# TencentARC/Mix-of-Show

Measured on AMD Instinct MI355X. Metric: edlora_train_images_per_sec_512_sd15, higher is better.
Workload: dtype fp16; 1 GPU; BASELINE.json configs[1]: single-concept ED-LoRA tune, SD-1.5 UNet/CLIP/VAE (random init, calibrated), 512x512, LoRA rank 4 on Attention+CLIPAttention, attn_reg on, batch 4/GPU; global_batch=4, per_gpu_batch=4, image_size=512, parallelism=dp1, grad_bucket_bytes=4466688, preset=sd15, hipgraph=True, channels_last=True

## Files before the change

### include/mos_hip.h

```cpp
#ifndef MOS_HIP_H
#define MOS_HIP_H

#include <stdint.h>

#ifdef __cplusplus
extern "C" {
#endif

typedef enum { MOS_F16 = 0, MOS_BF16 = 1 } mos_dtype;

typedef enum {
    MOS_OK = 0,
    MOS_ERR_BAD_ARG = -1,
    MOS_ERR_UNSUPPORTED = -2,
    MOS_ERR_LAUNCH = -3
} mos_status;

#define MOS_LORA_PAD 16
#define MOS_MAX_PCOLS 4
#define MOS_MAX_SOURCES 9

int mos_version(void);
const char* mos_last_error_string(void);

// ... 66 lines not shown
                              const void* A16T, const void* BpT,
                              void* dt, void* dx, int64_t lddx,
                              const mos_lora_grad_out* grads_host, void* ws,
                              int M, int N, int K, int lora_cols, int dtype, void* stream);

typedef struct {
    const float* partial[2];
    int C[2], cb[2];
    int nchunk, nj, block_begin, n_blocks;
    mos_lora_grad_out out;
} mos_lora_final_rec;
int mos_lora_linear_fused_bwd_deferred(const void* dy, int64_t lddy, const void* x, int64_t ldx,
                                       const void* Wt, int64_t ldwt, const void* t,
                                       const void* A16T, const void* BpT,
                                       void* dt, void* dx, int64_t lddx,
                                       const mos_lora_grad_out* grads_host, void* ws,
                                       int M, int N, int K, int lora_cols, int dtype, void* stream,
                                       mos_lora_final_rec* rec_host);
int mos_lora_grad_final_all(const mos_lora_final_rec* recs_dev, int n_recs, int total_blocks, void* stream);

typedef struct {
    const void* P[2];
    const void* Z[2];
    int64_t ldz[2];
    int C[2], cb[2];
    float* partial[2];
    int M, rpc, nchunk, nj;
    int block_begin, n_blocks;
    double flops, bytes;
} mos_lora_grad_job;
int mos_lora_linear_fused_bwd_deferred_all(const void* dy, int64_t lddy, const void* x, int64_t ldx,
                                           const void* Wt, int64_t ldwt, const void* t,
                                           const void* A16T, const void* BpT,
                                           void* dt, void* dx, int64_t lddx,
                                           const mos_lora_grad_out* grads_host, void* ws,
                                           int M, int N, int K, int lora_cols, int dtype, void* stream,
                                           mos_lora_final_rec* rec_host, mos_lora_grad_job* job_host);
int mos_lora_grad_all(const mos_lora_grad_job* jobs_dev, int n_jobs, int total_blocks, int nj, int dtype, double flops, double bytes,
                      void* stream);

typedef struct {
    int B, H, Nq, Nkv, d;
    int64_t q_bs, q_rs;
    int64_t k_bs, k_rs;
    int64_t v_bs, v_rs;
    int64_t o_bs, o_rs;
    float scale;
    int causal;
} mos_attn_shape;

int mos_attn_fwd(const void* q, const void* k, const void* v, void* o, float* lse,
                 const int32_t* tok_idx, int n_pcols, float* pcols,
                 const mos_attn_shape* shape_host, int dtype, void* stream);

typedef struct {
    int64_t do_bs, do_rs;
    int64_t dq_bs, dq_rs;
    int64_t dk_bs, dk_rs;
    int64_t dv_bs, dv_rs;
} mos_attn_grad_strides;

int64_t mos_attn_bwd_workspace_bytes(const mos_attn_shape* shape_host);
int mos_attn_bwd(const void* q, const void* k, const void* v, const void* o, const float* lse,
                 const void* dO, const int32_t* tok_idx, int n_pcols, const float* pcols,
                 const float* dpcols, void* dq, void* dk, void* dv, void* ws,
                 const mos_attn_shape* shape_host, const mos_attn_grad_strides* gs_host,
                 int dtype, void* stream);

int mos_self_attn_fwd(const void* q, const void* k, const void* v, void* o, float* lse,
                      const mos_attn_shape* shape_host, int dtype, void* stream);
int mos_cross_attn_fwd(const void* q, const void* k, const void* v, void* o, float* lse,
                       const int32_t* tok_idx, int n_pcols, float* pcols,
                       const mos_attn_shape* shape_host, int dtype, void* stream);
int mos_self_attn_bwd(const void* q, const void* k, const void* v, const void* o, const float* lse, const void* dO,
                      void* dq, void* dk, void* dv, void* ws, const mos_attn_shape* shape_host,
                      const mos_attn_grad_strides* gs_host, int dtype, void* stream);
int mos_cross_attn_bwd(const void* q, const void* k, const void* v, const void* o, const float* lse, const void* dO,
                       const int32_t* tok_idx, int n_pcols, const float* pcols, const float* dpcols,
                       void* dq, void* dk, void* dv, void* ws, const mos_attn_shape* shape_host,
                       const mos_attn_grad_strides* gs_host, int dtype, void* stream);

typedef struct {
    int n_regions;
    int feat_h, feat_w;
    int box[MOS_MAX_SOURCES - 1][4];
    int64_t src_stride;
} mos_region_desc;

int mos_region_cross_attn_fwd(const void* q, const void* k_src, const void* v_src, void* o,
                              const mos_attn_shape* shape_host, const mos_region_desc* reg_host,
                              int dtype, void* stream);
int mos_region_cross_attn_fwd_chunk(const void* q, const void* k_src, const void* v_src, void* o,
                                    const mos_attn_shape* shape_host, const mos_region_desc* reg_host,
                                    const void* total_count, int accumulate, int dtype, void* stream);

int mos_attn_probs(const void* q, const void* k, void* probs, const mos_attn_shape* shape_host, int dtype, void* stream);
int mos_attn_pv(const void* probs, const void* v, void* o, const mos_attn_shape* shape_host, int dtype, void* stream);
int64_t mos_attn_probs_bwd_workspace_bytes(const mos_attn_shape* shape_host);
int mos_attn_pv_bwd(const void* probs, const void* v, const void* dO, void* dprobs, void* dv, void* ws,
                    const mos_attn_shape* shape_host, const mos_attn_grad_strides* gs_host, int dtype, void* stream);
int mos_attn_probs_bwd(const void* q, const void* k, const void* probs, const void* dprobs, void* dq, void* dk, void* ws,
                       const mos_attn_shape* shape_host, const mos_attn_grad_strides* gs_host, int dtype, void* stream);

int64_t mos_gram_workspace_bytes(int64_t n, int Cin, int Cout);
int mos_gram_accumulate(const void* X, int64_t ldx, const void* Y, int64_t ldy, int64_t n,
                        int Cin, int Cout, int dtype, double* G, double* P, double* c,
// ... 68 lines not shown
```

### mix-of-show_amd/csrc/mos_attn.hip

```cpp
#include <cstdio>
#include <cstdlib>
#include <type_traits>
#include "mos_common.h"

#ifndef MOS_DQ_OCC
#define MOS_DQ_OCC 2
#endif
#ifndef MOS_ATTN_PV16
#define MOS_ATTN_PV16 1
#endif

namespace {

constexpr float LOG2E = 1.4426950408889634f;
constexpr float NEG_BIG = -1.0e30f;
constexpr int KV_TILE = 64;
constexpr int TS = KV_TILE + 8;
__device__ __forceinline__ constexpr int tr_col(int c) { return (c & ~12) | ((c & 4) << 1) | ((c & 8) >> 1); }

__device__ __forceinline__ constexpr int tr_col16(int c) {
    return (c & 32) | ((((c >> 2) & 1) * 2 + ((c >> 4) & 1)) << 3) | (((c >> 3) & 1) << 2) | (c & 3);
}

template <int D>
// ... 1391 lines not shown

template <int D> constexpr size_t fwd_lds(size_t es) { return 2 * (HD<D>::ROW_TILE_ELEMS + HD<D>::TR_TILE_ELEMS) * es; }
template <int D> constexpr size_t dq_lds(size_t es) { return 2 * (2 * HD<D>::ROW_TILE_ELEMS + HD<D>::TR_TILE_ELEMS) * es; }
template <int D> constexpr size_t dkdv_lds(size_t es) {
    return DKDV_NBUF<D>::value * ((2 * HD<D>::ROW_TILE_ELEMS + 2 * HD<D>::TR_TILE_ELEMS) * es +
                                  KV_TILE * (2 + MOS_MAX_PCOLS) * sizeof(float));
}

template <typename K>
void set_lds(K kernel, size_t bytes) {
    if (bytes > 48 * 1024)
        (void)hipFuncSetAttribute(reinterpret_cast<const void*>(kernel), hipFuncAttributeMaxDynamicSharedMemorySize, (int)bytes);
}

int check_shape(const mos_attn_shape* s, const char* who) {
    if (!s) return mos_set_error(MOS_ERR_BAD_ARG, "%s: NULL shape", who);
    if (s->B <= 0 || s->H <= 0 || s->Nq <= 0 || s->Nkv <= 0)
        return mos_set_error(MOS_ERR_BAD_ARG, "%s: B=%d H=%d Nq=%d Nkv=%d", who, s->B, s->H, s->Nq, s->Nkv);
    if (s->d != 40 && s->d != 64 && s->d != 80 && s->d != 160)
        return mos_set_error(MOS_ERR_UNSUPPORTED, "%s: head dim %d not in {40, 64, 80, 160}", who, s->d);
    if (s->causal && s->Nq != s->Nkv)
        return mos_set_error(MOS_ERR_BAD_ARG, "%s: causal masking needs Nq == Nkv (got %d, %d)", who, s->Nq, s->Nkv);
    if (s->q_rs % 8 || s->k_rs % 8 || s->v_rs % 8 || s->o_rs % 4 || s->q_bs % 8 || s->k_bs % 8 || s->v_bs % 8 || s->o_bs % 4)
        return mos_set_error(MOS_ERR_BAD_ARG, "%s: strides must be multiples of 8 elements", who);
    return MOS_OK;
}

AttnArgs make_args(const void* q, const void* k, const void* v, void* o, float* lse, const int32_t* tok, int np,
                   float* pcols, const mos_attn_shape* s, int q_tile) {
    AttnArgs a;
    a.q = q; a.k = k; a.v = v; a.o = o; a.lse = lse; a.tok_idx = tok; a.pcols = pcols; a.n_pcols = np;
    a.B = s->B; a.H = s->H; a.Nq = s->Nq; a.Nkv = s->Nkv; a.nqb = (s->Nq + q_tile - 1) / q_tile;
    a.q_bs = s->q_bs; a.q_rs = s->q_rs; a.k_bs = s->k_bs; a.k_rs = s->k_rs;
    a.v_bs = s->v_bs; a.v_rs = s->v_rs; a.o_bs = s->o_bs; a.o_rs = s->o_rs; a.scale = s->scale;
    a.causal = s->causal;
    return a;
}

template <typename T>
const char* tname() { return sizeof(T) == 2 && std::is_same<T, f16_t>::value ? "f16" : "bf16"; }

struct AttnKey {
    char s[96];
    double flops, bytes;
    AttnKey(const char* dt, const mos_attn_shape* sh, double gemms) {
        snprintf(s, sizeof(s), "%s d%d B%d H%d Nq%d Nkv%d", dt, sh->d, sh->B, sh->H, sh->Nq, sh->Nkv);
        flops = gemms * 2.0 * sh->B * sh->H * (double)sh->Nq * sh->Nkv * sh->d;
        bytes = 2.0 * sh->B * sh->H * sh->d * (2.0 * sh->Nq + 2.0 * sh->Nkv);
    }
};

template <int D> constexpr bool has_causal() { return true; }

template <typename T, int D, int QW, bool PCOLS, bool CAUSAL>
void launch_fwd_one(const AttnArgs& a, size_t lds, hipStream_t st) {
    const dim3 grid((unsigned)(a.H * a.nqb * a.B));
    set_lds(&attn_fwd_kernel<T, D, QW, PCOLS, CAUSAL>, lds);
    hipLaunchKernelGGL((attn_fwd_kernel<T, D, QW, PCOLS, CAUSAL>), grid, dim3(256), lds, st, a);
}
template <typename T, int D, int QW>
void launch_fwd_qw(const AttnArgs& a, int np, size_t lds, hipStream_t st) {
    if constexpr (has_causal<D>()) {
        if (a.causal) {
            if (np > 0) launch_fwd_one<T, D, QW, true, true>(a, lds, st);
            else launch_fwd_one<T, D, QW, false, true>(a, lds, st);
            return;
        }
    }
    if (np > 0) launch_fwd_one<T, D, QW, true, false>(a, lds, st);
    else launch_fwd_one<T, D, QW, false, false>(a, lds, st);
}

template <typename T, int D>
int launch_fwd(const void* q, const void* k, const void* v, void* o, float* lse, const int32_t* tok, int np,
               float* pcols, const mos_attn_shape* s, hipStream_t st) {
    constexpr int QW = fwd_qw<D>();
    const size_t lds = fwd_lds<D>(sizeof(T));
    AttnKey key(tname<T>(), s, 2.0);
    MosProfScope prof(st, np > 0 ? "attn_fwd_pcols" : "attn_fwd", key.s, key.flops, key.bytes);
    const int64_t wg_big = (int64_t)s->H * s->B * ((s->Nq + 4 * QW - 1) / (4 * QW));
    if (QW == 64 && wg_big < 512) {
        launch_fwd_qw<T, D, 32>(make_args(q, k, v, o, lse, tok, np, pcols, s, 128), np, lds, st);
    } else {
        launch_fwd_qw<T, D, QW>(make_args(q, k, v, o, lse, tok, np, pcols, s, 4 * QW), np, lds, st);
    }
    return mos_check_launch("attn_fwd");
}

template <typename T, int D>
int launch_region(const void* q, const void* k, const void* v, void* o, const mos_attn_shape* s,
                  const mos_region_desc* reg, const unsigned char* total_count, int accumulate, hipStream_t st) {
    AttnArgs a = make_args(q, k, v, o, nullptr, nullptr, 0, nullptr, s, 128);
    a.nqb = ((reg->feat_w + 15) / 16) * ((reg->feat_h + 7) / 8);
    const dim3 grid((unsigned)(a.H * a.nqb * a.B));
    const size_t lds = RG<D>::lds_bytes(sizeof(T));
    set_lds(&region_attn_kernel<T, D>, lds);
    double cover = 0.0, area = 0.0;
    for (int r = 0; r < reg->n_regions; ++r) {
        const double bh = reg->box[r][2] - reg->box[r][0], bw = reg->box[r][3] - reg->box[r][1];
        if (bh > 0 && bw > 0) area += bh * bw;
    }
    cover = area + (double)s->Nq;
    AttnKey key(tname<T>(), s, 2.0);
    char rk[128];
    snprintf(rk, sizeof(rk), "%s R%d", key.s, reg->n_regions);
    MosProfScope prof(st, "region_attn", rk, key.flops * cover / (double)s->Nq, key.bytes);
    hipLaunchKernelGGL((region_attn_kernel<T, D>), grid, dim3(256), lds, st, a, *reg, total_count, accumulate);
    return mos_check_launch("region_attn");
}

struct BwdPlan { int nw_q, nw_k, nqb, nkb, nsplit, q_per_split; };
BwdPlan plan_bwd(const mos_attn_shape* s) {
    BwdPlan p;
    p.nw_q = 4;
    p.nw_k = 4;
    p.nqb = (s->Nq + 32 * p.nw_q - 1) / (32 * p.nw_q);
    p.nkb = (s->Nkv + 32 * p.nw_k - 1) / (32 * p.nw_k);
    const int64_t base = (int64_t)p.nkb * s->B * s->H;
    const int qtiles = (s->Nq + KV_TILE - 1) / KV_TILE;
    int ns = (int)((512 + base - 1) / base);
    if (ns > qtiles) ns = qtiles;
    if (ns < 1) ns = 1;
    int tps = (qtiles + ns - 1) / ns;
    ns = (qtiles + tps - 1) / tps;
    p.nsplit = ns;
    p.q_per_split = tps * KV_TILE;
    return p;
}

template <typename T, int D>
int launch_bwd(const void* q, const void* k, const void* v, const void* o, const float* lse, const void* dO,
               const int32_t* tok, int np, const float* pcols, const float* dpcols, void* dq, void* dk, void* dv,
               void* ws, const mos_attn_shape* s, const mos_attn_grad_strides* g, hipStream_t st) {
    const BwdPlan p = plan_bwd(s);
    float* Dvec = (float*)ws;
    const int64_t nrows = (int64_t)s->B * s->H * s->Nq;
    float* part = Dvec + ((nrows + 3) / 4) * 4;
    AttnBwdArgs a;
    a.q = q; a.k = k; a.v = v; a.dO = dO; a.lse = lse; a.Dvec = Dvec; a.tok_idx = tok; a.dpcols = dpcols;
    a.o = o; a.o_bs = s->o_bs; a.o_rs = s->o_rs; a.pcols = pcols;
    a.n_pcols = (dpcols != nullptr && pcols != nullptr) ? np : 0;
    a.dq = dq; a.dk = dk; a.dv = dv; a.part = part;
    a.B = s->B; a.H = s->H; a.Nq = s->Nq; a.Nkv = s->Nkv; a.nqb = p.nqb; a.nkb = p.nkb;
    a.nsplit = p.nsplit; a.q_per_split = p.q_per_split;
    a.q_bs = s->q_bs; a.q_rs = s->q_rs; a.k_bs = s->k_bs; a.k_rs = s->k_rs; a.v_bs = s->v_bs; a.v_rs = s->v_rs;
    a.do_bs = g->do_bs; a.do_rs = g->do_rs; a.dq_bs = g->dq_bs; a.dq_rs = g->dq_rs;
    a.dk_bs = g->dk_bs; a.dk_rs = g->dk_rs; a.dv_bs = g->dv_bs; a.dv_rs = g->dv_rs; a.scale = s->scale;
    a.causal = s->causal;
    const bool pc = a.n_pcols > 0;
    {
        const dim3 grid((unsigned)(a.H * a.nqb * a.B));
        const size_t lds = dq_lds<D>(sizeof(T));
        AttnKey key(tname<T>(), s, 3.0);
        MosProfScope prof(st, "attn_bwd_dq", key.s, key.flops, key.bytes * 1.5);
        auto go = [&](auto pc_c, auto ca_c) {
            constexpr bool PC = decltype(pc_c)::value, CA = decltype(ca_c)::value;
            set_lds(&attn_bwd_dq_kernel<T, D, PC, 4, CA>, lds);
            hipLaunchKernelGGL((attn_bwd_dq_kernel<T, D, PC, 4, CA>), grid, dim3(256), lds, st, a);
        };
        bool done = false;
        if constexpr (has_causal<D>()) {
            if (a.causal) {
                if (pc) go(std::true_type{}, std::true_type{}); else go(std::false_type{}, std::true_type{});
                done = true;
            }
        }
        if (!done) { if (pc) go(std::true_type{}, std::false_type{}); else go(std::false_type{}, std::false_type{}); }
        int rc = mos_check_launch("attn_bwd_dq");
        if (rc) return rc;
    }
    {
        const dim3 grid((unsigned)(a.H * a.nkb * a.B), (unsigned)a.nsplit);
        const size_t lds = dkdv_lds<D>(sizeof(T));
        AttnKey key(tname<T>(), s, 4.0);
        MosProfScope prof(st, "attn_bwd_dkdv", key.s, key.flops, key.bytes * 1.5);
        auto go = [&](auto pc_c, auto ca_c) {
            constexpr bool PC = decltype(pc_c)::value, CA = decltype(ca_c)::value;
            set_lds(&attn_bwd_dkdv_kernel<T, D, PC, 4, CA>, lds);
            hipLaunchKernelGGL((attn_bwd_dkdv_kernel<T, D, PC, 4, CA>), grid, dim3(256), lds, st, a);
        };
        bool done = false;
        if constexpr (D == 40) {
            if (!pc && !a.causal && s->Nq % KV_TILE == 0 && a.q_per_split % KV_TILE == 0) {
                set_lds(&attn_bwd_dkdv_pipe_kernel<T, D>, lds);
                hipLaunchKernelGGL((attn_bwd_dkdv_pipe_kernel<T, D>), grid, dim3(256), lds, st, a);
                done = true;
            }
        }
        if constexpr (has_causal<D>()) {
            if (!done && a.causal) {
                if (pc) go(std::true_type{}, std::true_type{}); else go(std::false_type{}, std::true_type{});
                done = true;
            }
        }
        if (!done) { if (pc) go(std::true_type{}, std::false_type{}); else go(std::false_type{}, std::false_type{}); }
        int rc = mos_check_launch("attn_bwd_dkdv");
        if (rc) return rc;
    }
    if (a.nsplit > 1) {
        const int64_t slab4 = (int64_t)s->B * s->H * s->Nkv * D / 4;
        hipLaunchKernelGGL((attn_bwd_reduce_kernel<T, D>), dim3((unsigned)((slab4 + 255) / 256)), dim3(256), 0, st, part,
                           a.nsplit, (T*)dk, g->dk_bs, g->dk_rs, (T*)dv, g->dv_bs, g->dv_rs, s->B, s->H, s->Nkv);
        return mos_check_launch("attn_bwd_reduce");
    }
    return MOS_OK;
}

#define MOS_DISPATCH_TD(dtype, d, CALL)                                                     \
    do {                                                                                    \
        if ((dtype) == MOS_F16) {                                                           \
            typedef f16_t TT;                                                               \
            if ((d) == 40) { constexpr int DD = 40; return CALL; }                          \
            if ((d) == 64) { constexpr int DD = 64; return CALL; }                          \
            if ((d) == 80) { constexpr int DD = 80; return CALL; }                          \
            if ((d) == 160) { constexpr int DD = 160; return CALL; }                        \
        } else if ((dtype) == MOS_BF16) {                                                   \
            typedef bf16_t TT;                                                              \
            if ((d) == 40) { constexpr int DD = 40; return CALL; }                          \
            if ((d) == 64) { constexpr int DD = 64; return CALL; }                          \
            if ((d) == 80) { constexpr int DD = 80; return CALL; }                          \
            if ((d) == 160) { constexpr int DD = 160; return CALL; }                        \
        }                                                                                   \
        return mos_set_error(MOS_ERR_UNSUPPORTED, "unsupported dtype %d / head dim %d", (int)(dtype), (int)(d)); \
    } while (0)

}

extern "C" {

int mos_attn_fwd(const void* q, const void* k, const void* v, void* o, float* lse, const int32_t* tok_idx, int n_pcols,
                 float* pcols, const mos_attn_shape* s, int dtype, void* stream) {
    int rc = check_shape(s, "mos_attn_fwd");
    if (rc) return rc;
    MOS_REQUIRE(q && k && v && o, "mos_attn_fwd: NULL tensor");
    MOS_REQUIRE(n_pcols >= 0 && n_pcols <= MOS_MAX_PCOLS, "mos_attn_fwd: n_pcols=%d (max %d)", n_pcols, MOS_MAX_PCOLS);
    MOS_REQUIRE(n_pcols == 0 || (tok_idx && pcols), "mos_attn_fwd: n_pcols>0 needs tok_idx and pcols");
    hipStream_t st = (hipStream_t)stream;
    MOS_DISPATCH_TD(dtype, s->d, (launch_fwd<TT, DD>(q, k, v, o, lse, tok_idx, n_pcols, pcols, s, st)));
}

int mos_self_attn_fwd(const void* q, const void* k, const void* v, void* o, float* lse, const mos_attn_shape* s,
                      int dtype, void* stream) {
    return mos_attn_fwd(q, k, v, o, lse, nullptr, 0, nullptr, s, dtype, stream);
}

int mos_cross_attn_fwd(const void* q, const void* k, const void* v, void* o, float* lse, const int32_t* tok_idx,
                       int n_pcols, float* pcols, const mos_attn_shape* s, int dtype, void* stream) {
    return mos_attn_fwd(q, k, v, o, lse, tok_idx, n_pcols, pcols, s, dtype, stream);
}

int64_t mos_attn_bwd_workspace_bytes(const mos_attn_shape* s) {
    if (!s) return 0;
    const BwdPlan p = plan_bwd(s);
    const int64_t nrows = (int64_t)s->B * s->H * s->Nq;
    int64_t fl = ((nrows + 3) / 4) * 4;
    if (p.nsplit > 1) fl += 2 * (int64_t)p.nsplit * s->B * s->H * s->Nkv * s->d;
    return fl * (int64_t)sizeof(float);
}

int mos_attn_bwd(const void* q, const void* k, const void* v, const void* o, const float* lse, const void* dO,
                 const int32_t* tok_idx, int n_pcols, const float* pcols, const float* dpcols, void* dq, void* dk,
                 void* dv, void* ws, const mos_attn_shape* s, const mos_attn_grad_strides* g, int dtype, void* stream) {
    int rc = check_shape(s, "mos_attn_bwd");
    if (rc) return rc;
    MOS_REQUIRE(q && k && v && o && lse && dO && dq && dk && dv && ws && g, "mos_attn_bwd: NULL argument");
    MOS_REQUIRE(n_pcols >= 0 && n_pcols <= MOS_MAX_PCOLS, "mos_attn_bwd: n_pcols=%d", n_pcols);
    MOS_REQUIRE(dpcols == nullptr || (n_pcols > 0 && tok_idx && pcols), "mos_attn_bwd: dpcols needs tok_idx, pcols");
    MOS_REQUIRE(g->do_rs % 8 == 0 && g->dq_rs % 4 == 0 && g->dk_rs % 4 == 0 && g->dv_rs % 4 == 0,
                "mos_attn_bwd: gradient strides misaligned");
    hipStream_t st = (hipStream_t)stream;
    MOS_DISPATCH_TD(dtype, s->d,
                    (launch_bwd<TT, DD>(q, k, v, o, lse, dO, tok_idx, n_pcols, pcols, dpcols, dq, dk, dv, ws, s, g, st)));
}

int mos_self_attn_bwd(const void* q, const void* k, const void* v, const void* o, const float* lse, const void* dO, void* dq,
                      void* dk, void* dv, void* ws, const mos_attn_shape* s, const mos_attn_grad_strides* g, int dtype,
                      void* stream) {
    return mos_attn_bwd(q, k, v, o, lse, dO, nullptr, 0, nullptr, nullptr, dq, dk, dv, ws, s, g, dtype, stream);
}

int mos_cross_attn_bwd(const void* q, const void* k, const void* v, const void* o, const float* lse, const void* dO,
                       const int32_t* tok_idx, int n_pcols, const float* pcols, const float* dpcols, void* dq, void* dk,
                       void* dv, void* ws, const mos_attn_shape* s, const mos_attn_grad_strides* g, int dtype, void* stream) {
    return mos_attn_bwd(q, k, v, o, lse, dO, tok_idx, n_pcols, pcols, dpcols, dq, dk, dv, ws, s, g, dtype, stream);
}

int mos_region_cross_attn_fwd(const void* q, const void* k_src, const void* v_src, void* o, const mos_attn_shape* s,
                              const mos_region_desc* reg, int dtype, void* stream) {
    return mos_region_cross_attn_fwd_chunk(q, k_src, v_src, o, s, reg, nullptr, 0, dtype, stream);
}

int mos_region_cross_attn_fwd_chunk(const void* q, const void* k_src, const void* v_src, void* o, const mos_attn_shape* s,
                                    const mos_region_desc* reg, const void* total_count, int accumulate, int dtype,
                                    void* stream) {
    int rc = check_shape(s, "mos_region_cross_attn_fwd");
    MOS_REQUIRE(!accumulate || total_count, "mos_region_cross_attn_fwd_chunk: accumulate needs the total count map");
    if (rc) return rc;
    MOS_REQUIRE(q && k_src && v_src && o && reg, "mos_region_cross_attn_fwd: NULL argument");
    MOS_REQUIRE(reg->n_regions >= 0 && reg->n_regions <= MOS_MAX_SOURCES - 1, "mos_region_cross_attn_fwd: n_regions=%d",
                reg->n_regions);
    MOS_REQUIRE(reg->feat_h > 0 && reg->feat_w > 0 && reg->feat_h * reg->feat_w == s->Nq,
                "mos_region_cross_attn_fwd: feat %dx%d != Nq %d", reg->feat_h, reg->feat_w, s->Nq);
    if (s->Nkv <= 64 || s->Nkv > 96)
// ... 9 lines not shown
```

### mix-of-show_amd/mixofshow/hip/lib.py

```python
import ctypes
import os
import threading

_HERE = os.path.dirname(os.path.abspath(__file__))
LIB_PATH = os.environ.get('MOS_HIP_LIB') or os.path.normpath(os.path.join(_HERE, '..', '..', 'libmos_hip.so'))

MOS_F16 = 0
MOS_BF16 = 1
MOS_LORA_PAD = 16
MOS_MAX_PCOLS = 4
MOS_MAX_SOURCES = 9


class MosHipUnavailable(RuntimeError):
    pass


class MosHipError(RuntimeError):
    pass


class LoraSites(ctypes.Structure):
    _fields_ = [
        ('n_sites', ctypes.c_int),
# ... 62 lines not shown
        ('causal', ctypes.c_int),
    ]


class AttnGradStrides(ctypes.Structure):
    _fields_ = [
        ('do_bs', ctypes.c_int64), ('do_rs', ctypes.c_int64),
        ('dq_bs', ctypes.c_int64), ('dq_rs', ctypes.c_int64),
        ('dk_bs', ctypes.c_int64), ('dk_rs', ctypes.c_int64),
        ('dv_bs', ctypes.c_int64), ('dv_rs', ctypes.c_int64),
    ]


class RegionDesc(ctypes.Structure):
    _fields_ = [
        ('n_regions', ctypes.c_int),
        ('feat_h', ctypes.c_int), ('feat_w', ctypes.c_int),
        ('box', (ctypes.c_int * 4) * (MOS_MAX_SOURCES - 1)),
        ('src_stride', ctypes.c_int64),
    ]


_vp, _i, _i64, _f, _d = ctypes.c_void_p, ctypes.c_int, ctypes.c_int64, ctypes.c_float, ctypes.c_double

SIGNATURES = {
    'mos_version': (_i, []),
    'mos_last_error_string': (ctypes.c_char_p, []),
    'mos_profile_begin': (_i, []),
    'mos_profile_end': (_i, []),
    'mos_profile_get': (_i, [_i, ctypes.c_char_p, _i, ctypes.POINTER(ctypes.c_double),
                             ctypes.POINTER(ctypes.c_longlong), ctypes.POINTER(ctypes.c_double),
                             ctypes.POINTER(ctypes.c_double)]),
    'mos_lora_pack': (_i, [ctypes.POINTER(LoraSites), _i, _vp, _vp, _vp, _vp, _vp]),
    'mos_lora_pack_all': (_i, [_vp, _i, _i, _i, _vp]),
    'mos_lora_linear_fused_fwd': (_i, [_vp, _i64, _vp, _i64, _vp, _vp, _vp, _vp, _i64, _vp, _i, _i, _i, _i, _vp]),
    'mos_lora_linear_fwd_ex': (_i, [_vp, _i64, _vp, _i64, _vp, _vp, _vp, _vp, _i64, _vp, _i, _i, _i, _i,
                                    ctypes.POINTER(GemmEpilogue), _vp]),
    'mos_lora_linear_fused_bwd': (_i, [_vp, _i64, _vp, _i64, _vp, _i64, _vp, _vp, _vp, _vp, _vp, _i64,
                                       ctypes.POINTER(LoraGradOut), _vp, _i, _i, _i, _i, _i, _vp]),
    'mos_lora_linear_fused_bwd_deferred': (_i, [_vp, _i64, _vp, _i64, _vp, _i64, _vp, _vp, _vp, _vp, _vp, _i64,
                                                ctypes.POINTER(LoraGradOut), _vp, _i, _i, _i, _i, _i, _vp,
                                                ctypes.POINTER(LoraFinalRec)]),
    'mos_lora_linear_fused_bwd_deferred_all': (_i, [_vp, _i64, _vp, _i64, _vp, _i64, _vp, _vp, _vp, _vp, _vp, _i64,
                                                ctypes.POINTER(LoraGradOut), _vp, _i, _i, _i, _i, _i, _vp,
                                                ctypes.POINTER(LoraFinalRec), ctypes.POINTER(LoraGradJob)]),
    'mos_lora_grad_all': (_i, [_vp, _i, _i, _i, _i, ctypes.c_double, ctypes.c_double, _vp]),
    'mos_lora_grad_final_all': (_i, [_vp, _i, _i, _vp]),
    'mos_lora_down': (_i, [_vp, _i64, _vp, _vp, _i, _i, _i, _vp]),
    'mos_lora_linear_fwd': (_i, [_vp, _i64, _vp, _i64, _vp, _vp, _vp, _vp, _i64, _i, _i, _i, _i, _vp]),
    'mos_lora_bwd_workspace_bytes': (_i64, [_i, _i, _i]),
    'mos_lora_linear_bwd': (_i, [_vp, _i64, _vp, _i64, _vp, _i64, _vp, _vp, _vp, _vp, _vp, _i64, _vp, _vp, _vp,
                                 _i, _i, _i, _i, _i, _vp]),
    'mos_attn_fwd': (_i, [_vp, _vp, _vp, _vp, _vp, _vp, _i, _vp, ctypes.POINTER(AttnShape), _i, _vp]),
    'mos_attn_bwd_workspace_bytes': (_i64, [ctypes.POINTER(AttnShape)]),
    'mos_attn_bwd': (_i, [_vp, _vp, _vp, _vp, _vp, _vp, _vp, _i, _vp, _vp, _vp, _vp, _vp, _vp,
                          ctypes.POINTER(AttnShape), ctypes.POINTER(AttnGradStrides), _i, _vp]),
    'mos_self_attn_fwd': (_i, [_vp, _vp, _vp, _vp, _vp, ctypes.POINTER(AttnShape), _i, _vp]),
    'mos_cross_attn_fwd': (_i, [_vp, _vp, _vp, _vp, _vp, _vp, _i, _vp, ctypes.POINTER(AttnShape), _i, _vp]),
    'mos_region_cross_attn_fwd': (_i, [_vp, _vp, _vp, _vp, ctypes.POINTER(AttnShape), ctypes.POINTER(RegionDesc),
                                       _i, _vp]),
    'mos_region_cross_attn_fwd_chunk': (_i, [_vp, _vp, _vp, _vp, ctypes.POINTER(AttnShape), ctypes.POINTER(RegionDesc),
                                             _vp, _i, _i, _vp]),
    'mos_attn_probs': (_i, [_vp, _vp, _vp, ctypes.POINTER(AttnShape), _i, _vp]),
    'mos_attn_pv': (_i, [_vp, _vp, _vp, ctypes.POINTER(AttnShape), _i, _vp]),
    'mos_attn_probs_bwd_workspace_bytes': (_i64, [ctypes.POINTER(AttnShape)]),
    'mos_attn_pv_bwd': (_i, [_vp, _vp, _vp, _vp, _vp, _vp, ctypes.POINTER(AttnShape), ctypes.POINTER(AttnGradStrides), _i, _vp]),
    'mos_attn_probs_bwd': (_i, [_vp, _vp, _vp, _vp, _vp, _vp, _vp, ctypes.POINTER(AttnShape), ctypes.POINTER(AttnGradStrides),
                                _i, _vp]),
    'mos_self_attn_bwd': (_i, [_vp, _vp, _vp, _vp, _vp, _vp, _vp, _vp, _vp, _vp, ctypes.POINTER(AttnShape),
                               ctypes.POINTER(AttnGradStrides), _i, _vp]),
    'mos_cross_attn_bwd': (_i, [_vp, _vp, _vp, _vp, _vp, _vp, _vp, _i, _vp, _vp, _vp, _vp, _vp, _vp, ctypes.POINTER(AttnShape),
                                ctypes.POINTER(AttnGradStrides), _i, _vp]),
    'mos_gram_workspace_bytes': (_i64, [_i64, _i, _i]),
    'mos_gram_accumulate': (_i, [_vp, _i64, _vp, _i64, _i64, _i, _i, _i, _vp, _vp, _vp, _vp, _vp]),
    'mos_groupnorm_workspace_bytes': (_i64, [_i, _i, _i, _i]),
    'mos_groupnorm_silu_fwd': (_i, [_vp, _vp, _vp, _vp, _vp, _vp, _i, _i, _i, _i, _f, _i, _i, _vp]),
    'mos_groupnorm_silu_bwd': (_i, [_vp, _vp, _vp, _vp, _vp, _vp, _vp, _i, _i, _i, _i, _i, _i, _vp]),
    'mos_groupnorm_nhwc_workspace_bytes': (_i64, [_i, _i, _i, _i]),
    'mos_groupnorm_silu_fwd_nhwc': (_i, [_vp, _vp, _vp, _vp, _vp, _vp, _i, _i, _i, _i, _f, _i, _i, _vp]),
    'mos_groupnorm_silu_bwd_nhwc': (_i, [_vp, _vp, _vp, _vp, _vp, _vp, _vp, _i, _i, _i, _i, _i, _i, _vp]),
    'mos_groupnorm_silu_bwd_nhwc_res_ps': (_i, [_vp, _vp, _i64, _vp, _vp, _vp, _vp, _vp, _vp, _i, _i, _i, _i, _i, _i, _vp]),
    'mos_groupnorm_silu_bwd_nhwc_res': (_i, [_vp, _vp, _vp, _vp, _vp, _vp, _vp, _vp, _i, _i, _i, _i, _i, _i, _vp]),
    'mos_conv3x3_nhwc': (_i, [_vp, _vp, _vp, _vp, _vp, _vp, _i, _i, _i, _i, _i, _i, _i, _vp]),
    'mos_conv3x3_nhwc_workspace_bytes': (_i64, [_i, _i, _i, _i, _i]),
    'mos_conv3x3_gn_tiles': (_i, [_i, _i, _i, _i, _i]),
    'mos_conv3x3_nhwc_px': (_i, [_vp, _i64, _vp, _vp, _vp, _vp, _vp, _i, _i, _i, _i, _i, _i, _i, _vp, _vp, _vp]),
    'mos_conv3x3_nhwc_gn': (_i, [_vp, _vp, _vp, _vp, _vp, _vp, _i, _i, _i, _i, _i, _i, _i, _vp, _vp, _vp]),
    'mos_groupnorm_nhwc_reads_twice': (_i, [_i, _i, _i, _i]),
    'mos_groupnorm_silu_fwd_nhwc_pre': (_i, [_vp, _vp, _i, _vp, _vp, _vp, _vp, _vp, _i, _i, _i, _i, _f, _i, _i, _vp]),
    'mos_conv3x3_s2_nhwc': (_i, [_vp, _vp, _vp, _vp, _i, _i, _i, _i, _i, _i, _i, _vp, _vp]),
    'mos_conv3x3_nhwc_ws': (_i, [_vp, _vp, _vp, _vp, _vp, _vp, _i, _i, _i, _i, _i, _i, _i, _vp, _vp]),
    'mos_layernorm_fwd': (_i, [_vp, _vp, _vp, _vp, _vp, _i, _i, _f, _i, _vp]),
    'mos_layernorm_bwd': (_i, [_vp, _vp, _vp, _vp, _vp, _i, _i, _i, _vp]),
    'mos_add_layernorm_fwd': (_i, [_vp, _vp, _vp, _vp, _vp, _vp, _vp, _i, _i, _f, _i, _i, _vp]),
    'mos_add_layernorm_bwd': (_i, [_vp, _vp, _vp, _vp, _vp, _vp, _vp, _i, _i, _i, _i, _vp]),
    'mos_geglu_fwd': (_i, [_vp, _vp, _i64, _i, _i, _vp]),
    'mos_softmax_rows': (_i, [_vp, _vp, _i, _i, _f, _i, _vp]),
    'mos_geglu_bwd': (_i, [_vp, _vp, _vp, _i64, _i, _i, _vp]),
    'mos_quick_gelu_fwd': (_i, [_vp, _vp, _i64, _i, _vp]),
    'mos_quick_gelu_bwd': (_i, [_vp, _vp, _vp, _i64, _i, _vp]),
    'mos_lsq_workspace_bytes': (_i64, [_i, _i]),
    'mos_lsq_loss_grad_gram': (_i, [_vp, _vp, _vp, _vp, _d, _i, _i, _vp, _vp, _vp, _vp]),
}

_lib = None
_lock = threading.Lock()
# ... 30 lines not shown
```

### mix-of-show_amd/mixofshow/hip/ops.py

```python
import ctypes

import torch

from . import lib as _lib
from .lib import MOS_BF16, MOS_F16, MOS_LORA_PAD, MOS_MAX_PCOLS, MOS_MAX_SOURCES

_DT = {torch.float16: MOS_F16, torch.bfloat16: MOS_BF16}


def _dt(t):
    try:
        return _DT[t.dtype]
    except KeyError:
        raise TypeError(f'mixofshow.hip: dtype {t.dtype} not supported by the HIP kernels (float16 / bfloat16 only)')


def _dev(*ts):
    for t in ts:
        if t is not None and not t.is_cuda:
            raise RuntimeError('mixofshow.hip: kernel-backed ops need tensors on a HIP device (cuda:N); got '
                               f'{t.device}. There is no CPU fallback in the product path.')


def _stream():
# ... 191 lines not shown
        assert bias.dtype == torch.float32 and bias.is_contiguous()
    epi = _lib.GemmEpilogue()
    epi.residual, epi.ldr = None, 0
    if residual is not None:
        assert residual.shape == (M, N) and residual.dtype == x.dtype
        epi.residual, epi.ldr = residual.data_ptr(), _rows(residual)
    y = torch.empty((M, N), dtype=x.dtype, device=x.device)
    t = torch.empty((M, MOS_LORA_PAD), dtype=x.dtype, device=x.device) if (need_t and A16 is not None) else None
    L = _lib.load()
    _lib.check(L.mos_lora_linear_fwd_ex(_p(x), _rows(x), _p(W), _rows(W), _p(A16), _p(Bp16), _p(bias), _p(y), _rows(y), _p(t),
                                        M, N, K, _dt(x), ctypes.byref(epi), _stream()), 'mos_lora_linear_fwd_ex')
    return y, t


def linear_bwd(dy, x, Wt, t, A16T, BpT, need_dx=True, need_lora=True, lora_cols=16):
    _dev(dy, x, Wt, t, A16T, BpT)
    M, N = dy.shape
    lora = BpT is not None
    K = Wt.shape[0] if Wt is not None else x.shape[1]
    dev = dy.device
    dx = torch.empty((M, K), dtype=dy.dtype, device=dev) if need_dx else None
    dt = torch.empty((M, MOS_LORA_PAD), dtype=dy.dtype, device=dev) if lora else None
    dA16 = torch.empty((MOS_LORA_PAD, K), dtype=torch.float32, device=dev) if (lora and need_lora) else None
    dBpT = torch.empty((MOS_LORA_PAD, N), dtype=torch.float32, device=dev) if (lora and need_lora) else None
    L = _lib.load()
    ws = None
    if lora:
        ws = torch.empty((L.mos_lora_bwd_workspace_bytes(M, N, K) + 3) // 4, dtype=torch.float32, device=dev)
    _lib.check(L.mos_lora_linear_bwd(_p(dy), _rows(dy), _p(x), _rows(x) if x is not None else 0,
                                     _p(Wt), _rows(Wt) if Wt is not None else 0, _p(t), _p(A16T), _p(BpT),
                                     _p(dt), _p(dx), _rows(dx) if dx is not None else 0, _p(dA16), _p(dBpT), _p(ws),
                                     M, N, K, int(lora_cols), _dt(dy), _stream()), 'mos_lora_linear_bwd')
    return dx, dA16, dBpT


def _attn_view(t):
    assert t.dim() == 3 and t.stride(2) == 1, f'need (B, N, C) with contiguous channels, got strides {t.stride()}'
    return t.stride(0), t.stride(1)


def _shape(q, k, v, o, heads, scale, causal=False):
    B, Nq, C = q.shape
    s = _lib.AttnShape()
    s.B, s.H, s.Nq, s.Nkv, s.d = B, heads, Nq, k.shape[1], C // heads
    s.q_bs, s.q_rs = _attn_view(q)
    s.k_bs, s.k_rs = _attn_view(k)
    s.v_bs, s.v_rs = _attn_view(v)
    s.o_bs, s.o_rs = _attn_view(o)
    s.scale = float(scale)
    s.causal = int(bool(causal))
    return s


def attn_fwd(q, k, v, heads, scale, tok_idx=None, need_lse=True, causal=False):
    _dev(q, k, v, tok_idx)
    B, Nq, C = q.shape
    o = torch.empty((B, Nq, C), dtype=q.dtype, device=q.device)
    s = _shape(q, k, v, o, heads, scale, causal)
    lse = torch.empty((B, heads, Nq), dtype=torch.float32, device=q.device) if need_lse else None
    T = 0
    pcols = None
    if tok_idx is not None:
        assert tok_idx.dtype == torch.int32 and tok_idx.is_contiguous() and tok_idx.shape[0] == B
        T = tok_idx.shape[1]
        assert 1 <= T <= MOS_MAX_PCOLS
        pcols = torch.empty((B, heads, Nq, T), dtype=torch.float32, device=q.device)
    L = _lib.load()
    _lib.check(L.mos_attn_fwd(_p(q), _p(k), _p(v), _p(o), _p(lse), _p(tok_idx), T, _p(pcols), ctypes.byref(s),
                              _dt(q), _stream()), 'mos_attn_fwd')
    return o, lse, pcols


def attn_bwd(q, k, v, o, lse, dO, heads, scale, dq, dk, dv, tok_idx=None, pcols=None, dpcols=None, causal=False):
    _dev(q, k, v, o, lse, dO, dq, dk, dv, tok_idx, pcols, dpcols)
    s = _shape(q, k, v, o, heads, scale, causal)
    g = _lib.AttnGradStrides()
    g.do_bs, g.do_rs = _attn_view(dO)
    g.dq_bs, g.dq_rs = _attn_view(dq)
    g.dk_bs, g.dk_rs = _attn_view(dk)
    g.dv_bs, g.dv_rs = _attn_view(dv)
    T = tok_idx.shape[1] if tok_idx is not None else 0
    if dpcols is not None:
        assert dpcols.dtype == torch.float32 and dpcols.is_contiguous() and pcols is not None
    L = _lib.load()
    ws = torch.empty((L.mos_attn_bwd_workspace_bytes(ctypes.byref(s)) + 3) // 4, dtype=torch.float32, device=q.device)
    _lib.check(L.mos_attn_bwd(_p(q), _p(k), _p(v), _p(o), _p(lse), _p(dO), _p(tok_idx), T, _p(pcols), _p(dpcols),
                              _p(dq), _p(dk), _p(dv), _p(ws), ctypes.byref(s), ctypes.byref(g), _dt(q), _stream()),
               'mos_attn_bwd')
    return dq, dk, dv


_region_count_cache = {}


def region_total_count(boxes, feat_h, feat_w, device):
    key = (tuple(tuple(int(v) for v in b) for b in boxes), int(feat_h), int(feat_w), str(device))
    t = _region_count_cache.get(key)
    if t is None:
        cnt = torch.zeros((feat_h, feat_w), dtype=torch.int32)
        for h0, w0, h1, w1 in key[0]:
            if h1 > h0 and w1 > w0:
                cnt[max(h0, 0):h1, max(w0, 0):w1] += 1
        assert int(cnt.max()) <= 255, 'more than 255 overlapping regions on one query'
        if len(_region_count_cache) > 256:
            _region_count_cache.clear()
        t = _region_count_cache[key] = cnt.to(torch.uint8).reshape(-1).to(device)
# ... 371 lines not shown
```

Baseline: 131.3 images/s.

## Add single-block attention kernels for short sequences with head dim 64

Adds specialized forward and backward attention kernels for head dim 64 with Nq, Nkv ≤ 96 (e.g. the CLIP text encoder at 77 tokens). Each block handles a whole (batch, head) and stages K/V (or Q/dO/K) once in LDS. The backward pass fuses the D-vector, dK/dV and dQ computation into one launch instead of several kernels plus workspace. The aim is to cut launch count and tiling overhead for tiny attention. The cost is a larger LDS footprint and an extra code path, which covers only shapes without pcols.

```diff
diff --git a/include/mos_hip.h b/include/mos_hip.h
--- a/include/mos_hip.h
+++ b/include/mos_hip.h
@@ -142,6 +142,8 @@
 int mos_attn_fwd(const void* q, const void* k, const void* v, void* o, float* lse,
                  const int32_t* tok_idx, int n_pcols, float* pcols,
                  const mos_attn_shape* shape_host, int dtype, void* stream);
+
+int mos_attn_small_form(const mos_attn_shape* shape_host, int n_pcols);
 
 typedef struct {
     int64_t do_bs, do_rs;
diff --git a/mix-of-show_amd/csrc/mos_attn.hip b/mix-of-show_amd/csrc/mos_attn.hip
--- a/mix-of-show_amd/csrc/mos_attn.hip
+++ b/mix-of-show_amd/csrc/mos_attn.hip
@@ -1467,6 +1467,8 @@
 
 template <int D> constexpr bool has_causal() { return true; }
 
+#include "mos_attn_small.inc"
+
 template <typename T, int D, int QW, bool PCOLS, bool CAUSAL>
 void launch_fwd_one(const AttnArgs& a, size_t lds, hipStream_t st) {
     const dim3 grid((unsigned)(a.H * a.nqb * a.B));
@@ -1490,6 +1492,9 @@
 int launch_fwd(const void* q, const void* k, const void* v, void* o, float* lse, const int32_t* tok, int np,
                float* pcols, const mos_attn_shape* s, hipStream_t st) {
     constexpr int QW = fwd_qw<D>();
+    if constexpr (D == SM::D) {
+        if (small_form(s, np)) return launch_small_fwd<T>(make_args(q, k, v, o, lse, tok, np, pcols, s, SM::NMAX), s, st);
+    }
     const size_t lds = fwd_lds<D>(sizeof(T));
     AttnKey key(tname<T>(), s, 2.0);
     MosProfScope prof(st, np > 0 ? "attn_fwd_pcols" : "attn_fwd", key.s, key.flops, key.bytes);
@@ -1563,6 +1568,9 @@
     a.dk_bs = g->dk_bs; a.dk_rs = g->dk_rs; a.dv_bs = g->dv_bs; a.dv_rs = g->dv_rs; a.scale = s->scale;
     a.causal = s->causal;
     const bool pc = a.n_pcols > 0;
+    if constexpr (D == SM::D) {
+        if (small_form(s, a.n_pcols)) return launch_small_bwd<T>(a, s, st);
+    }
     {
         const dim3 grid((unsigned)(a.H * a.nqb * a.B));
         const size_t lds = dq_lds<D>(sizeof(T));
@@ -1664,6 +1672,11 @@
     return mos_attn_fwd(q, k, v, o, lse, tok_idx, n_pcols, pcols, s, dtype, stream);
 }
 
+int mos_attn_small_form(const mos_attn_shape* s, int n_pcols) {
+    if (!s) return 0;
+    return small_form(s, n_pcols) ? 1 : 0;
+}
+
 int64_t mos_attn_bwd_workspace_bytes(const mos_attn_shape* s) {
     if (!s) return 0;
     const BwdPlan p = plan_bwd(s);
diff --git a/mix-of-show_amd/csrc/mos_attn_small.inc b/mix-of-show_amd/csrc/mos_attn_small.inc
--- /dev/null
+++ b/mix-of-show_amd/csrc/mos_attn_small.inc
@@ -0,0 +1,342 @@
+#ifndef MOS_ATTN_SMALL
+#define MOS_ATTN_SMALL 1
+#endif
+
+struct SM {
+    static constexpr int D = 64;
+    static constexpr int NMAX = 96;
+    static constexpr int NT = 192;
+    static constexpr int RS = HD<D>::RS;
+    static constexpr int TS3 = NMAX + 8;
+    static constexpr int ROW_ELEMS = NMAX * RS;
+    static constexpr int TR_ELEMS = D * TS3;
+    static constexpr int DCH = D / 8;
+    static constexpr int NROW = NMAX * DCH / NT;
+    static constexpr int NTR = NMAX / 2 * DCH / NT;
+    static constexpr size_t fwd_lds(size_t es) { return (size_t)(ROW_ELEMS + TR_ELEMS) * es; }
+    static constexpr size_t bwd_lds(size_t es) { return (size_t)(2 * ROW_ELEMS + 3 * TR_ELEMS) * es + 2 * NMAX * sizeof(float); }
+};
+static_assert(SM::NMAX * SM::DCH % SM::NT == 0 && SM::NMAX / 2 * SM::DCH % SM::NT == 0, "staging items divide evenly");
+static_assert(SM::NMAX * SM::TS3 <= 2 * SM::ROW_ELEMS, "the dS image fits over the Q and dO row images");
+
+template <typename T>
+struct SmallStage {
+    u32x4 r0[SM::NTR], r1[SM::NTR];
+    __device__ __forceinline__ void load(rsrc_t src, int64_t rs, int tid) {
+#pragma unroll
+        for (int i = 0; i < SM::NTR; ++i) {
+            const int it = tid + SM::NT * i;
+            const int pr = it % (SM::NMAX / 2), ch = it / (SM::NMAX / 2);
+            const int off = (2 * pr * (int)rs + ch * 8) * (int)sizeof(T);
+            r0[i] = ldbuf16(src, off);
+            r1[i] = ldbuf16(src, off + (int)rs * (int)sizeof(T));
+        }
+    }
+    __device__ __forceinline__ void store_rows(T* lds, int tid) const {
+#pragma unroll
+        for (int i = 0; i < SM::NTR; ++i) {
+            const int it = tid + SM::NT * i;
+            const int pr = it % (SM::NMAX / 2), ch = it / (SM::NMAX / 2);
+            st16(lds + (2 * pr) * SM::RS + ch * 8, r0[i]);
+            st16(lds + (2 * pr + 1) * SM::RS + ch * 8, r1[i]);
+        }
+    }
+    __device__ __forceinline__ void store_tr(T* ldsT, int tid) const {
+#pragma unroll
+        for (int i = 0; i < SM::NTR; ++i) {
+            const int it = tid + SM::NT * i;
+            const int pr = it % (SM::NMAX / 2), ch = it / (SM::NMAX / 2);
+            uint32_t* dst = reinterpret_cast<uint32_t*>(ldsT + (ch * 8) * SM::TS3 + tr_col(2 * pr));
+#pragma unroll
+            for (int w = 0; w < 4; ++w) {
+                dst[(2 * w) * (SM::TS3 / 2)] = __builtin_amdgcn_perm(r1[i][w], r0[i][w], 0x05040100u);
+                dst[(2 * w + 1) * (SM::TS3 / 2)] = __builtin_amdgcn_perm(r1[i][w], r0[i][w], 0x07060302u);
+            }
+        }
+    }
+};
+
+template <typename T, bool CAUSAL>
+__global__ __launch_bounds__(SM::NT, 3) void attn_small_fwd_kernel(AttnArgs a) {
+    typedef typename MT<T>::v8 v8;
+    constexpr int D = SM::D, KS = HD<D>::KS, DT = HD<D>::DT, RS = SM::RS, TS3 = SM::TS3;
+    extern __shared__ __attribute__((aligned(16))) unsigned char smem_raw[];
+    T* Vt = reinterpret_cast<T*>(smem_raw);
+    T* Ks = Vt + SM::TR_ELEMS;
+    const int tid = threadIdx.x, lane = tid & 63, wave = tid >> 6, l31 = lane & 31, hh = lane >> 5;
+    const int h = blockIdx.x % a.H, b = blockIdx.x / a.H;
+    const int q0 = 32 * wave, qi = q0 + l31;
+
+    const T* qp = (const T*)a.q + (int64_t)b * a.q_bs + h * D;
+    const rsrc_t ksrc = make_rsrc((const T*)a.k + (int64_t)b * a.k_bs + h * D, slice_bytes<T, D>(a.Nkv, a.k_rs));
+    const rsrc_t vsrc = make_rsrc((const T*)a.v + (int64_t)b * a.v_bs + h * D, slice_bytes<T, D>(a.Nkv, a.v_rs));
+    u32x4 kr[SM::NROW];
+#pragma unroll
+    for (int i = 0; i < SM::NROW; ++i) {
+        const int cc = tid + SM::NT * i;
+        kr[i] = ldbuf16(ksrc, ((cc / SM::DCH) * (int)a.k_rs + (cc % SM::DCH) * 8) * (int)sizeof(T));
+    }
+    SmallStage<T> vst;
+    vst.load(vsrc, a.v_rs, tid);
+    v8 qf[KS];
+    load_row_frags<T, D>(qf, qp + (int64_t)min(qi, a.Nq - 1) * a.q_rs, qi < a.Nq, hh);
+#pragma unroll
+    for (int i = 0; i < SM::NROW; ++i) {
+        const int cc = tid + SM::NT * i;
+        st16(Ks + (cc / SM::DCH) * RS + (cc % SM::DCH) * 8, kr[i]);
+    }
+    vst.store_tr(Vt, tid);
+    __syncthreads();
+    if (q0 >= a.Nq) return;
+
+    int nt = (a.Nkv + 31) >> 5;
+    if (CAUSAL) nt = min(nt, wave + 1);
+    f32x16 sT[3];
+#pragma unroll
+    for (int t = 0; t < 3; ++t) {
+        if (t < nt) {
+#pragma unroll
+            for (int r = 0; r < 16; ++r) sT[t][r] = 0.f;
+#pragma unroll
+            for (int ks = 0; ks < KS; ++ks) {
+                const v8 af = as_v8<T>(ld16(Ks + (32 * t + l31) * RS + ks * 16 + hh * 8));
+                sT[t] = MT<T>::mfma32(af, qf[ks], sT[t]);
+            }
+#pragma unroll
+            for (int r = 0; r < 16; ++r) {
+                const int key = 32 * t + acc_row(r, hh);
+                if (key >= a.Nkv || (CAUSAL && key > qi)) sT[t][r] = NEG_BIG;
+            }
+        } else {
+#pragma unroll
+            for (int r = 0; r < 16; ++r) sT[t][r] = NEG_BIG;
+        }
+    }
+    const float c = a.scale * LOG2E;
+    float mx = NEG_BIG;
+#pragma unroll
+    for (int t = 0; t < 3; ++t)
+#pragma unroll
+        for (int r = 0; r < 16; ++r) mx = fmaxf(mx, sT[t][r]);
+    mx = fmaxf(mx, __shfl_xor(mx, 32));
+    const float mc = mx * c;
+    float ls = 0.f;
+#pragma unroll
+    for (int t = 0; t < 3; ++t)
+#pragma unroll
+        for (int r = 0; r < 16; ++r) {
+            const float p = __builtin_amdgcn_exp2f(sT[t][r] * c - mc);
+            sT[t][r] = p;
+            ls += p;
+        }
+    const float lt = ls + __shfl_xor(ls, 32);
+    f32x16 o[DT];
+#pragma unroll
+    for (int dt = 0; dt < DT; ++dt)
+#pragma unroll
+        for (int r = 0; r < 16; ++r) o[dt][r] = 0.f;
+#pragma unroll
+    for (int t = 0; t < 3; ++t) {
+        if (t < nt) {
+#pragma unroll
+            for (int s2 = 0; s2 < 2; ++s2) {
+                if (32 * t + 16 * s2 >= a.Nkv) continue;
+                const v8 pf = acc_to_bfrag<T>(sT[t], s2);
+#pragma unroll
+                for (int dt = 0; dt < DT; ++dt)
+                    o[dt] = MT<T>::mfma32(tr_afrag<T>(Vt + (32 * dt + l31) * TS3, t, s2, hh), pf, o[dt]);
+            }
+        }
+    }
+    T* op = (T*)a.o + (int64_t)b * a.o_bs + h * D;
+    store_out_rows<T, D>(op + (int64_t)qi * a.o_rs, qi < a.Nq, o, 1.0f / lt, hh);
+    if (a.lse != nullptr && hh == 0 && qi < a.Nq) a.lse[((int64_t)b * a.H + h) * a.Nq + qi] = mx * a.scale + __logf(lt);
+}
+
+template <typename T, bool CAUSAL>
+__global__ __launch_bounds__(SM::NT, 2) void attn_small_bwd_kernel(AttnBwdArgs a) {
+    typedef typename MT<T>::v8 v8;
+    constexpr int D = SM::D, KS = HD<D>::KS, DT = HD<D>::DT, RS = SM::RS, TS3 = SM::TS3;
+    extern __shared__ __attribute__((aligned(16))) unsigned char smem_raw[];
+    T* Qs = reinterpret_cast<T*>(smem_raw);
+    T* dOs = Qs + SM::ROW_ELEMS;
+    T* Qt = dOs + SM::ROW_ELEMS;
+    T* dOt = Qt + SM::TR_ELEMS;
+    T* Kt = dOt + SM::TR_ELEMS;
+    float* lse_s = reinterpret_cast<float*>(Kt + SM::TR_ELEMS);
+    float* nD_s = lse_s + SM::NMAX;
+    T* dSq = Qs;
+    const int tid = threadIdx.x, lane = tid & 63, wave = tid >> 6, l31 = lane & 31, hh = lane >> 5;
+    const int h = blockIdx.x % a.H, b = blockIdx.x / a.H;
+    const int k0 = 32 * wave, kvi = k0 + l31;
+    const bool kvalid = kvi < a.Nkv;
+
+    const T* qp = (const T*)a.q + (int64_t)b * a.q_bs + h * D;
+    const T* kp = (const T*)a.k + (int64_t)b * a.k_bs + h * D;
+    const T* vp = (const T*)a.v + (int64_t)b * a.v_bs + h * D;
+    const T* dop = (const T*)a.dO + (int64_t)b * a.do_bs + h * D;
+    const T* op = (const T*)a.o + (int64_t)b * a.o_bs + h * D;
+    const int64_t rowbase = ((int64_t)b * a.H + h) * a.Nq;
+
+    SmallStage<T> qst, dost, kst;
+    qst.load(make_rsrc(qp, slice_bytes<T, D>(a.Nq, a.q_rs)), a.q_rs, tid);
+    dost.load(make_rsrc(dop, slice_bytes<T, D>(a.Nq, a.do_rs)), a.do_rs, tid);
+    kst.load(make_rsrc(kp, slice_bytes<T, D>(a.Nkv, a.k_rs)), a.k_rs, tid);
+    v8 kf[KS], vf[KS];
+    load_row_frags<T, D>(kf, kp + (int64_t)min(kvi, a.Nkv - 1) * a.k_rs, kvalid, hh);
+    load_row_frags<T, D>(vf, vp + (int64_t)min(kvi, a.Nkv - 1) * a.v_rs, kvalid, hh);
+    if (tid < SM::NMAX) {
+        const bool qv = tid < a.Nq;
+        const int qc = min(tid, a.Nq - 1);
+        const T* orow = op + (int64_t)qc * a.o_rs;
+        const T* dorow = dop + (int64_t)qc * a.do_rs;
+        float d0 = 0.f, d1 = 0.f;
+#pragma unroll
+        for (int ks = 0; ks < KS; ++ks) {
+            const v8 o0 = as_v8<T>(ld16(orow + ks * 16)), g0 = as_v8<T>(ld16(dorow + ks * 16));
+            const v8 o1 = as_v8<T>(ld16(orow + ks * 16 + 8)), g1 = as_v8<T>(ld16(dorow + ks * 16 + 8));
+#pragma unroll
+            for (int e = 0; e < 8; ++e) {
+                d0 += (float)o0[e] * (float)g0[e];
+                d1 += (float)o1[e] * (float)g1[e];
+            }
+        }
+        lse_s[tid] = qv ? a.lse[rowbase + qc] * LOG2E : 0.f;
+        nD_s[tid] = qv ? -(d0 + d1) : 0.f;
+    }
+    qst.store_rows(Qs, tid);
+    dost.store_rows(dOs, tid);
+    qst.store_tr(Qt, tid);
+    dost.store_tr(dOt, tid);
+    kst.store_tr(Kt, tid);
+    __syncthreads();
+
+    const float c = a.scale * LOG2E;
+    f32x16 dkT[DT], dvT[DT];
+#pragma unroll
+    for (int dt = 0; dt < DT; ++dt)
+#pragma unroll
+        for (int r = 0; r < 16; ++r) { dkT[dt][r] = 0.f; dvT[dt][r] = 0.f; }
+    v8 dsf[3][2];
+    const bool wave_keys = k0 < a.Nkv;
+#pragma unroll
+    for (int t = 0; t < 3; ++t) {
+        const bool run = wave_keys && 32 * t < a.Nq && (!CAUSAL || t >= wave);
+        if (run) {
+            v8 aq[KS], ado[KS];
+#pragma unroll
+            for (int ks = 0; ks < KS; ++ks) {
+                const int off = (32 * t + l31) * RS + ks * 16 + hh * 8;
+                aq[ks] = as_v8<T>(ld16(Qs + off));
+                ado[ks] = as_v8<T>(ld16(dOs + off));
+            }
+            f32x4 l4[4];
+            f32x16 s, dp;
+#pragma unroll
+            for (int r4 = 0; r4 < 4; ++r4) {
+                const int ql = 32 * t + 8 * r4 + 4 * hh;
+                l4[r4] = *reinterpret_cast<const f32x4*>(lse_s + ql);
+                const f32x4 dd = *reinterpret_cast<const f32x4*>(nD_s + ql);
+#pragma unroll
+                for (int rr = 0; rr < 4; ++rr) { dp[4 * r4 + rr] = dd[rr]; s[4 * r4 + rr] = 0.f; }
+            }
+#pragma unroll
+            for (int ks = 0; ks < KS; ++ks) {
+                s = MT<T>::mfma32(aq[ks], kf[ks], s);
+                dp = MT<T>::mfma32(ado[ks], vf[ks], dp);
+            }
+#pragma unroll
+            for (int r4 = 0; r4 < 4; ++r4)
+#pragma unroll
+                for (int rr = 0; rr < 4; ++rr) {
+                    const int r = 4 * r4 + rr;
+                    float p = __builtin_amdgcn_exp2f(s[r] * c - l4[r4][rr]);
+                    if (!kvalid || (CAUSAL && kvi > 32 * t + 8 * r4 + 4 * hh + rr)) p = 0.f;
+                    s[r] = p;
+                    dp[r] = p * dp[r];
+                }
+            v8 pf[2];
+            pf[0] = acc_to_bfrag<T>(s, 0); pf[1] = acc_to_bfrag<T>(s, 1);
+            dsf[t][0] = acc_to_bfrag<T>(dp, 0); dsf[t][1] = acc_to_bfrag<T>(dp, 1);
+#pragma unroll
+            for (int dt = 0; dt < DT; ++dt)
+#pragma unroll
+                for (int s2 = 0; s2 < 2; ++s2) {
+                    dvT[dt] = MT<T>::mfma32(tr_afrag<T>(dOt + (32 * dt + l31) * TS3, t, s2, hh), pf[s2], dvT[dt]);
+                    dkT[dt] = MT<T>::mfma32(tr_afrag<T>(Qt + (32 * dt + l31) * TS3, t, s2, hh), dsf[t][s2], dkT[dt]);
+                }
+        } else {
+            dsf[t][0] = as_v8<T>(u32x4{0, 0, 0, 0});
+            dsf[t][1] = as_v8<T>(u32x4{0, 0, 0, 0});
+        }
+    }
+    if (wave_keys) {
+        store_out_rows<T, D>((T*)a.dk + (int64_t)b * a.dk_bs + (int64_t)kvi * a.dk_rs + h * D, kvalid, dkT, a.scale, hh);
+        store_out_rows<T, D>((T*)a.dv + (int64_t)b * a.dv_bs + (int64_t)kvi * a.dv_rs + h * D, kvalid, dvT, 1.0f, hh);
+    }
+    __syncthreads();
+
+    {
+        T* col = dSq + tr_col(kvi);
+#pragma unroll
+        for (int t = 0; t < 3; ++t)
+#pragma unroll
+            for (int s2 = 0; s2 < 2; ++s2)
+#pragma unroll
+                for (int j = 0; j < 8; ++j) col[(32 * t + acc_row(8 * s2 + j, hh)) * TS3] = dsf[t][s2][j];
+    }
+    __syncthreads();
+
+    if (k0 >= a.Nq) return;
+    const int qi = kvi;
+    f32x16 dq[DT];
+#pragma unroll
+    for (int dt = 0; dt < DT; ++dt)
+#pragma unroll
+        for (int r = 0; r < 16; ++r) dq[dt][r] = 0.f;
+#pragma unroll
+    for (int t = 0; t < 3; ++t) {
+        if (32 * t < a.Nkv && (!CAUSAL || t <= wave)) {
+#pragma unroll
+            for (int s2 = 0; s2 < 2; ++s2) {
+                const v8 bf = as_v8<T>(ld16(dSq + qi * TS3 + 32 * t + 16 * s2 + 8 * hh));
+#pragma unroll
+                for (int dt = 0; dt < DT; ++dt)
+                    dq[dt] = MT<T>::mfma32(tr_afrag<T>(Kt + (32 * dt + l31) * TS3, t, s2, hh), bf, dq[dt]);
+            }
+        }
+    }
+    store_out_rows<T, D>((T*)a.dq + (int64_t)b * a.dq_bs + (int64_t)qi * a.dq_rs + h * D, qi < a.Nq, dq, a.scale, hh);
+}
+
+inline bool small_form(const mos_attn_shape* s, int n_pcols) {
+    return MOS_ATTN_SMALL != 0 && s->d == SM::D && s->Nq >= 1 && s->Nkv >= 1 && s->Nq <= SM::NMAX && s->Nkv <= SM::NMAX &&
+           n_pcols == 0 && (!s->causal || s->Nq == s->Nkv);
+}
+
+template <typename T>
+int launch_small_fwd(const AttnArgs& a, const mos_attn_shape* s, hipStream_t st) {
+    const size_t lds = SM::fwd_lds(sizeof(T));
+    AttnKey key(tname<T>(), s, 2.0);
+    MosProfScope prof(st, "attn_fwd", key.s, key.flops, key.bytes);
+    const dim3 grid((unsigned)(a.H * a.B));
+    if (a.causal) hipLaunchKernelGGL((attn_small_fwd_kernel<T, true>), grid, dim3(SM::NT), lds, st, a);
+    else hipLaunchKernelGGL((attn_small_fwd_kernel<T, false>), grid, dim3(SM::NT), lds, st, a);
+    return mos_check_launch("attn_small_fwd");
+}
+
+template <typename T>
+int launch_small_bwd(const AttnBwdArgs& a, const mos_attn_shape* s, hipStream_t st) {
+    const size_t lds = SM::bwd_lds(sizeof(T));
+    AttnKey key(tname<T>(), s, 5.0);
+    MosProfScope prof(st, "attn_bwd", key.s, key.flops, key.bytes * 2.0);
+    const dim3 grid((unsigned)(a.H * a.B));
+    if (a.causal) {
+        set_lds(&attn_small_bwd_kernel<T, true>, lds);
+        hipLaunchKernelGGL((attn_small_bwd_kernel<T, true>), grid, dim3(SM::NT), lds, st, a);
+    } else {
+        set_lds(&attn_small_bwd_kernel<T, false>, lds);
+        hipLaunchKernelGGL((attn_small_bwd_kernel<T, false>), grid, dim3(SM::NT), lds, st, a);
+    }
+    return mos_check_launch("attn_small_bwd");
+}
diff --git a/mix-of-show_amd/mixofshow/hip/lib.py b/mix-of-show_amd/mixofshow/hip/lib.py
--- a/mix-of-show_amd/mixofshow/hip/lib.py
+++ b/mix-of-show_amd/mixofshow/hip/lib.py
@@ -138,6 +138,7 @@
     'mos_lora_linear_bwd': (_i, [_vp, _i64, _vp, _i64, _vp, _i64, _vp, _vp, _vp, _vp, _vp, _i64, _vp, _vp, _vp,
                                  _i, _i, _i, _i, _i, _vp]),
     'mos_attn_fwd': (_i, [_vp, _vp, _vp, _vp, _vp, _vp, _i, _vp, ctypes.POINTER(AttnShape), _i, _vp]),
+    'mos_attn_small_form': (_i, [ctypes.POINTER(AttnShape), _i]),
     'mos_attn_bwd_workspace_bytes': (_i64, [ctypes.POINTER(AttnShape)]),
     'mos_attn_bwd': (_i, [_vp, _vp, _vp, _vp, _vp, _vp, _vp, _i, _vp, _vp, _vp, _vp, _vp, _vp,
                           ctypes.POINTER(AttnShape), ctypes.POINTER(AttnGradStrides), _i, _vp]),
diff --git a/mix-of-show_amd/mixofshow/hip/ops.py b/mix-of-show_amd/mixofshow/hip/ops.py
--- a/mix-of-show_amd/mixofshow/hip/ops.py
+++ b/mix-of-show_amd/mixofshow/hip/ops.py
@@ -267,6 +267,11 @@
     return s
 
 
+def attn_small_form(q, k, v, heads, causal=False, n_pcols=0):
+    s = _shape(q, k, v, q, heads, 1.0, causal)
+    return int(_lib.load().mos_attn_small_form(ctypes.byref(s), int(n_pcols)))
+
+
 def attn_fwd(q, k, v, heads, scale, tok_idx=None, need_lse=True, causal=False):
     _dev(q, k, v, tok_idx)
     B, Nq, C = q.shape
```

Result: no change. 132.5 images/s, median of 6 (+0.9%).
